# sony/aki

Hardware: AMD Instinct MI355X
Metric: image+text tokens/sec forward, AKI-4B, 336px img + 512 txt (higher is better)
Workload: dtype bf16

## Files before the change

### aki_amd/build.py

```python
from __future__ import annotations

import argparse
import concurrent.futures as cf
import os
import subprocess
import sys

PKG = os.path.dirname(os.path.abspath(__file__))
ROOT = os.path.dirname(PKG)
CSRC = os.path.join(PKG, "csrc")
LIBDIR = os.path.join(PKG, "lib")
LIB = os.path.join(LIBDIR, "libaki_mi355x.so")
LAB_LIB = os.path.join(LIBDIR, "libaki_mi355x_lab.so")
LAB_SOURCES = ["api.hip", "gemm_bf16.hip", "gemm_tn_bf16.hip", "mma_attn_bf16.hip", "mma_attn64_bf16.hip", "decode_chain.hip"]
LAB_ONLY_SOURCES = []
SOURCES = ["api.hip", "gemm_bf16.hip", "gemm_tn_bf16.hip", "mma_attn_bf16.hip", "mma_attn64_bf16.hip", "attn_nc_bf16.hip", "decode.hip", "decode_chain.hip", "train_kernels.hip", "attn_bwd_bf16.hip", "fp8_quant.hip", "simple_f32.hip", "aux_kernels.hip", "stack.hip"]
ARCH = "gfx950"
FILE_FLAGS = {"mma_attn64_bf16.hip": ["-fno-slp-vectorize"]}


def csrc_hash() -> str:
    import hashlib
    h = hashlib.sha256()
    files = sorted(os.path.join(CSRC, f) for f in os.listdir(CSRC) if f.endswith((".hip", ".h"))) + [os.path.join(ROOT, "include", "aki_mi355x.h")]
    for f in files:
        h.update(os.path.basename(f).encode())
        h.update(open(f, "rb").read())
    return h.hexdigest()[:16]


def _hipcc() -> str:
    for c in (os.environ.get("HIPCC"), "/opt/rocm/bin/hipcc", "hipcc"):
        if c and (os.path.isabs(c) and os.path.exists(c) or not os.path.isabs(c)):
            return c
    return "hipcc"


def _newer(target: str, deps) -> bool:
    if not os.path.exists(target):
        return False
    t = os.path.getmtime(target)
    return all(os.path.getmtime(d) <= t for d in deps)


def build(force: bool = False, save_temps: bool = False, verbose: bool = True, lab: bool = True) -> str:
    os.makedirs(LIBDIR, exist_ok=True)
    objdir = os.path.join(LIBDIR, "obj")
    os.makedirs(objdir, exist_ok=True)
    headers = [os.path.join(CSRC, "aki_device.h"), os.path.join(CSRC, "attn_mma_common.h"), os.path.join(ROOT, "include", "aki_mi355x.h")]
    srcs = [os.path.join(CSRC, s) for s in SOURCES]
    lab_only = [os.path.join(CSRC, s_) for s_ in LAB_ONLY_SOURCES]
    if not force and _newer(LIB, srcs + headers) and (not lab or _newer(LAB_LIB, srcs + lab_only + headers)):
        return LIB
    flags = [f"--offload-arch={ARCH}", "-O3", "-fPIC", "-std=c++17", "-I", os.path.join(ROOT, "include"), "-I", CSRC,
             "-Wno-unused-result", "-ffp-contract=off"]
    if save_temps:
        flags += ["-save-temps=obj", "-Rpass-analysis=kernel-resource-usage"]

    def cc(job):
        src, is_lab = job
        obj = os.path.join(objdir, os.path.basename(src).replace(".hip", ".lab.o" if is_lab else ".o"))
        if not force and _newer(obj, [src] + headers):
            return obj, ""
        extra = (["-DAKI_LAB_HOOKS"] if is_lab else []) + FILE_FLAGS.get(os.path.basename(src), [])
        r = subprocess.run([_hipcc()] + flags + extra + ["-c", src, "-o", obj], capture_output=True, text=True)
        if r.returncode != 0:
            raise RuntimeError(f"hipcc failed for {src}:\n{r.stdout}\n{r.stderr}")
        return obj, r.stderr

    jobs = [(s_, False) for s_ in srcs] + ([(os.path.join(CSRC, s_), True) for s_ in LAB_SOURCES + LAB_ONLY_SOURCES] if lab else [])
    with cf.ThreadPoolExecutor(max_workers=min(4, len(jobs))) as ex:
        results = list(ex.map(cc, jobs))
    objs = [o for o, _ in results[:len(srcs)]]
    lab_objs = [o for o, _ in results[len(srcs):]]
    if verbose:
        for _, log in results:
            if log.strip():
                sys.stderr.write(log)
    r = subprocess.run([_hipcc(), f"--offload-arch={ARCH}", "-shared", "-fPIC", "-o", LIB] + objs, capture_output=True, text=True)
    if r.returncode != 0:
        raise RuntimeError(f"link failed:\n{r.stdout}\n{r.stderr}")
    if lab:
        swapped = {os.path.basename(o).replace(".lab.o", ".o"): o for o in lab_objs}
        mix = [swapped.pop(os.path.basename(o), o) for o in objs] + list(swapped.values())
        r = subprocess.run([_hipcc(), f"--offload-arch={ARCH}", "-shared", "-fPIC", "-o", LAB_LIB] + mix, capture_output=True, text=True)
        if r.returncode != 0:
            raise RuntimeError(f"link (lab) failed:\n{r.stdout}\n{r.stderr}")
    return LIB


if __name__ == "__main__":
    ap = argparse.ArgumentParser()
    ap.add_argument("--force", action="store_true")
    ap.add_argument("--save-temps", action="store_true")
    ap.add_argument("--no-lab", action="store_true", help="skip libaki_mi355x_lab.so")
    a = ap.parse_args()
    print(build(force=a.force, save_temps=a.save_temps, lab=not a.no_lab))
```

### aki_amd/csrc/attn_mma_common.h

```cpp
#pragma once
#include <type_traits>

#include "aki_device.h"

namespace aki {

struct AttnParams {
  const bf16_t* q;
  const bf16_t* k;
  const bf16_t* v;
  bf16_t* o;
  float* lse;
  const aki_mma_rect* rects;
  const uint64_t* vbits;
  const int* seq_lens;
  int max_rects;
  int B, H, L;
  int nqt, nwords;
  int splits;
  int group_bh;
  int kvcap;
  float scale_log2;
  int dead_uniform;
};

constexpr int KROW = 192;
constexpr int VROW = 192;
constexpr int KTILE = 64 * KROW;
constexpr int VTILE = 64 * VROW;
constexpr int NSTAGE = 3;

constexpr int MAX_VB_WORDS = 256;

__device__ __forceinline__ float max3(float a, float b, float c) {
  float r;
  asm("v_max3_f32 %0, %1, %2, %3" : "=v"(r) : "v"(a), "v"(b), "v"(c));
  return r;
}

__device__ __forceinline__ float tile_max32(const f32x16& s0, const f32x16& s1) {
  float m, m1, m2, m3;
  asm("v_max3_f32 %0, %4, %5, %6\n\tv_max3_f32 %1, %7, %8, %9\n\tv_max3_f32 %2, %10, %11, %12\n\tv_max3_f32 %3, %13, %14, %15\n\t"
      "v_max3_f32 %0, %0, %16, %17\n\tv_max3_f32 %1, %1, %18, %19\n\tv_max3_f32 %2, %2, %20, %21\n\tv_max3_f32 %3, %3, %22, %23"
      : "=&v"(m), "=&v"(m1), "=&v"(m2), "=&v"(m3)
      : "v"(s0[0]), "v"(s0[1]), "v"(s1[0]), "v"(s0[4]), "v"(s0[5]), "v"(s1[4]), "v"(s0[8]), "v"(s0[9]), "v"(s1[8]), "v"(s0[12]), "v"(s0[13]), "v"(s1[12]),
        "v"(s1[1]), "v"(s0[2]), "v"(s1[5]), "v"(s0[6]), "v"(s1[9]), "v"(s0[10]), "v"(s1[13]), "v"(s0[14]));
  asm("v_max3_f32 %0, %0, %4, %5\n\tv_max3_f32 %1, %1, %6, %7\n\tv_max3_f32 %2, %2, %8, %9\n\tv_max3_f32 %3, %3, %10, %11\n\t"
      "v_max3_f32 %0, %0, %12, %13\n\tv_max3_f32 %2, %2, %14, %15\n\tv_max3_f32 %0, %0, %1, %2\n\tv_max_f32 %0, %0, %3"
      : "+v"(m), "+v"(m1), "+v"(m2), "+v"(m3)
      : "v"(s0[3]), "v"(s1[2]), "v"(s0[7]), "v"(s1[6]), "v"(s0[11]), "v"(s1[10]), "v"(s0[15]), "v"(s1[14]),
        "v"(s1[3]), "v"(s1[7]), "v"(s1[11]), "v"(s1[15]));
  return m;
}

__device__ __forceinline__ int count_le(int x) {
  const int n = 4 * (x >> 3) + min((x & 7) + 1, 4);
  return x < 0 ? 0 : min(n, 32);
}

__device__ __forceinline__ unsigned low_bits(int n) { return n >= 32 ? ~0u : ((1u << n) - 1u); }

template <int BIT>
__device__ __forceinline__ float mask_bias(int hid, int ninf) {
  float b;
  asm("v_bfe_i32 %0, %1, %2, 1\n\tv_and_b32 %0, %3, %0" : "=&v"(b) : "v"(hid), "n"(BIT), "s"(ninf));
  return b;
}

template <int BIT0, int BIT1>
__device__ __forceinline__ void mask_bias2(int hid, int ninf, float& b0, float& b1) {
  asm volatile("v_bfe_i32 %0, %2, %3, 1\n\tv_bfe_i32 %1, %2, %4, 1\n\tv_and_b32 %0, %5, %0\n\tv_and_b32 %1, %5, %1"
               : "=&v"(b0), "=&v"(b1) : "v"(hid), "n"(BIT0), "n"(BIT1), "s"(ninf));
}

template <int N, class F>
__device__ __forceinline__ void static_for(F&& f) {
  if constexpr (N > 0) {
    static_for<N - 1>(f);
    f(std::integral_constant<int, N - 1>{});
  }
}

template <int OFF>
__device__ __forceinline__ u32x2 ds_read_tr(unsigned lds_addr) {
  u32x2 r;
  asm volatile("ds_read_b64_tr_b16 %0, %1 offset:%2" : "=v"(r) : "v"(lds_addr), "n"(OFF));
  return r;
}

}
```

### aki_amd/csrc/mma_attn64_bf16.hip

```cpp
#include "attn_mma_common.h"

namespace aki {

constexpr int A64_O = 64;
constexpr int A64_Q = 160;
constexpr int A64_KA = 208;
constexpr int A64_KC = 232;
constexpr int A64_L = 56;

template <int R> __device__ __forceinline__ void acc_zero() { asm volatile("v_accvgpr_write_b32 a%c0, 0" ::"n"(R)); }
template <int R> __device__ __forceinline__ void acc_set(unsigned x) { asm volatile("v_accvgpr_write_b32 a%c1, %0" ::"v"(x), "n"(R)); }
template <int R> __device__ __forceinline__ float acc_get() {
  float x;
  asm volatile("v_accvgpr_read_b32 %0, a%c1" : "=v"(x) : "n"(R));
  return x;
}
template <int R> __device__ __forceinline__ void acc_scale4(float alpha) {
  float t0, t1, t2, t3;
  asm volatile(
      "v_accvgpr_read_b32 %0, a%c5\n\tv_accvgpr_read_b32 %1, a%c6\n\tv_accvgpr_read_b32 %2, a%c7\n\tv_accvgpr_read_b32 %3, a%c8\n\t"
      "v_mul_f32 %0, %0, %4\n\tv_mul_f32 %1, %1, %4\n\tv_mul_f32 %2, %2, %4\n\tv_mul_f32 %3, %3, %4\n\t"
      "v_accvgpr_write_b32 a%c5, %0\n\tv_accvgpr_write_b32 a%c6, %1\n\tv_accvgpr_write_b32 a%c7, %2\n\tv_accvgpr_write_b32 a%c8, %3"
      : "=&v"(t0), "=&v"(t1), "=&v"(t2), "=&v"(t3)
      : "v"(alpha), "n"(R), "n"(R + 1), "n"(R + 2), "n"(R + 3));
// ... 246 lines not shown
  const float m = tile_max32(s0, s1);
  const float mx = halves_max(m) * c + X.hide;
  const float m_new = fmaxf(X.m_ref, mx);
  const float alpha = __builtin_amdgcn_exp2f(X.m_ref - m_new);
  const bool started = __ballot(X.m_ref > -1e29f) != 0ull;
  X.m_ref = m_new;
  if (started) {
    {
      float lt;
      asm volatile("v_accvgpr_read_b32 %0, a%c2\n\ts_nop 0\n\tv_mul_f32 %0, %0, %1\n\ts_nop 0\n\tv_accvgpr_write_b32 a%c2, %0" : "=&v"(lt) : "v"(alpha), "n"(A64_L + 4 * ((OA - A64_O) / 48)));
    }
    static_for<12>([&](auto I) { acc_scale4<OA + 4 * decltype(I)::value>(alpha); });
  }
  const float nm = -m_new + X.hide;
#pragma unroll
  for (int r = 0; r < 16; r += 2) {
    const float a = __builtin_amdgcn_exp2f(__builtin_fmaf(s0[r], c, nm)), b = __builtin_amdgcn_exp2f(__builtin_fmaf(s0[r + 1], c, nm));
    const float d = __builtin_amdgcn_exp2f(__builtin_fmaf(s1[r], c, nm)), e = __builtin_amdgcn_exp2f(__builtin_fmaf(s1[r + 1], c, nm));
    const unsigned w0 = pack_bf16x2(a, b), w1 = pack_bf16x2(d, e);
    pin(w0, w1);
    pf[r >> 3][(r & 7) >> 1] = w0;
    pf[2 + (r >> 3)][(r & 7) >> 1] = w1;
  }
}
template <int THR, int ABL>
__global__ __launch_bounds__(256, 1) void mma_attn64_bf16_kernel(const AttnParams p) {
  constexpr int NT = 256;
  constexpr int OROW = 208;
  constexpr int LDS_RING = NSTAGE * KTILE + NSTAGE * VTILE, LDS_VB = MAX_VB_WORDS * 8, LDS_OUT = 8 * 32 * OROW;
  __shared__ __attribute__((aligned(16))) char smem[LDS_RING + LDS_VB + LDS_OUT + 16];
  char* const sK = smem;
  char* const sV = smem + NSTAGE * KTILE;
  const unsigned sVB_a = (unsigned)(unsigned long)((__attribute__((address_space(3))) char*)(smem + NSTAGE * KTILE + NSTAGE * VTILE));
  if constexpr (THR != 0) asm volatile("" ::: "a56", "a57", "a58", "a59", "a60", "a61", "a62", "a63");
  asm volatile("" ::: "a64", "a65", "a66", "a67", "a68", "a69", "a70", "a71", "a72", "a73", "a74", "a75", "a76", "a77", "a78", "a79", "a80", "a81", "a82", "a83", "a84", "a85", "a86", "a87", "a88", "a89", "a90", "a91", "a92", "a93", "a94", "a95", "a96", "a97", "a98", "a99", "a100", "a101", "a102", "a103", "a104", "a105", "a106", "a107", "a108", "a109", "a110", "a111", "a112", "a113", "a114", "a115", "a116", "a117", "a118", "a119", "a120", "a121", "a122", "a123", "a124", "a125", "a126", "a127", "a128", "a129", "a130", "a131", "a132", "a133", "a134", "a135", "a136", "a137", "a138", "a139", "a140", "a141", "a142", "a143", "a144", "a145", "a146", "a147", "a148", "a149", "a150", "a151", "a152", "a153", "a154", "a155", "a156", "a157", "a158", "a159", "a160", "a161", "a162", "a163", "a164", "a165", "a166", "a167", "a168", "a169", "a170", "a171", "a172", "a173", "a174", "a175", "a176", "a177", "a178", "a179", "a180", "a181", "a182", "a183", "a184", "a185", "a186", "a187", "a188", "a189", "a190", "a191", "a192", "a193", "a194", "a195", "a196", "a197", "a198", "a199", "a200", "a201", "a202", "a203", "a204", "a205", "a206", "a207", "a208", "a209", "a210", "a211", "a212", "a213", "a214", "a215", "a216", "a217", "a218", "a219", "a220", "a221", "a222", "a223", "a224", "a225", "a226", "a227", "a228", "a229", "a230", "a231", "a232", "a233", "a234", "a235", "a236", "a237", "a238", "a239", "a240", "a241", "a242", "a243", "a244", "a245", "a246", "a247", "a248", "a249", "a250", "a251", "a252", "a253", "a254", "a255");

  const int tid = threadIdx.x, lane = tid & 63;
  const int wave = __builtin_amdgcn_readfirstlane(tid >> 6);
  const int l31 = lane & 31, h = lane >> 5;
  const unsigned ones_w = (((lane & 7) == 0 && ((lane >> 4) & 1) == 0) || ((lane & 7) == 4 && ((lane >> 4) & 1) == 1)) ? 0x3f803f80u : 0u;
  const u32x4 sel = {ones_w, ones_w, ones_w, ones_w};
  const unsigned sFlag_a = (unsigned)(unsigned long)((__attribute__((address_space(3))) char*)(smem + LDS_RING + LDS_VB + LDS_OUT));
  if constexpr (THR != 0) {
    if (tid == 0) { *(unsigned*)(smem + LDS_RING + LDS_VB + LDS_OUT) = 0u; *(unsigned*)(smem + LDS_RING + LDS_VB + LDS_OUT + 4) = 0u; }
  }
  bool force_checked = false;
  int vpar = 0;

  const int grp = blockIdx.x / (p.group_bh * p.splits);
  const int bh0 = grp * p.group_bh;
  const int gbh = min(p.group_bh, p.B * p.H - bh0);
  const int within = blockIdx.x - bh0 * p.splits;
  const int sidx = within / gbh;
  const int bh = bh0 + within - sidx * gbh;
  const int b = bh / p.H, head = bh - b * p.H;
  const int L = p.L;
  const bf16_t* qb = p.q + ((size_t)bh * L) * 96;
  const char* kb = (const char*)(p.k + ((size_t)bh * p.kvcap) * 96);
  const char* vb_ = (const char*)(p.v + ((size_t)bh * p.kvcap) * 96);
  const int Lb = p.seq_lens ? min(p.seq_lens[b], L) : L;

  int d_ko[3];
#pragma unroll
  for (int i = 0; i < 3; ++i) {
    const int ch = i * NT + tid;
    const int kr = ch / 12, pos = ch - kr * 12;
    d_ko[i] = kr * 192 + (pos ^ ((kr >> 2) & 3)) * 16;
  }
  const int d_vo = tid * 16;
  const __amdgpu_buffer_rsrc_t rsrc_k = __builtin_amdgcn_make_buffer_rsrc((void*)kb, 0, L * 192, 0x00020000);
  const __amdgpu_buffer_rsrc_t rsrc_v = __builtin_amdgcn_make_buffer_rsrc((void*)vb_, 0, L * 192, 0x00020000);
  auto dma_k = [&](auto I, int t, int st) {
    constexpr int i = decltype(I)::value;
    if constexpr (ABL & 2) return;
    __builtin_amdgcn_raw_ptr_buffer_load_lds(rsrc_k, AKI_LDS_PTR(sK + st * KTILE + (i * NT + wave * 64) * 16), 16, d_ko[i], t * 12288, 0, 0);
  };
  auto dma_v = [&](auto I, int t, int st) {
    constexpr int i = decltype(I)::value;
    if constexpr (ABL & 2) return;
    __builtin_amdgcn_raw_ptr_buffer_load_lds(rsrc_v, AKI_LDS_PTR(sV + st * VTILE + (i * NT + wave * 64) * 16), 16, d_vo, t * 12288 + i * 4096, 0, 0);
  };

  int first_bad = 0x7fffffff;
  {
    unsigned long long bad = 0ull;
    int base = 0;
#pragma unroll
    for (int q4 = 3; q4 >= 0; --q4) {
      const int w = lane + 64 * q4;
      unsigned long long vbw = ~0ull;
      if (w < p.nwords) {
        if (p.vbits) vbw = p.vbits[(size_t)b * p.nwords + w];
        else vbw = (w * 64 + 64 <= L) ? ~0ull : ((1ull << (L - w * 64)) - 1ull);
        if (wave == 0) *(unsigned long long*)(smem + NSTAGE * KTILE + NSTAGE * VTILE + 8 * w) = vbw;
      }
      const unsigned long long m = __ballot(vbw != ~0ull);
      if (m != 0ull) { bad = m; base = 64 * q4; }
    }
    if (bad != 0ull) first_bad = base + __builtin_ctzll(bad);
    __syncthreads();
  }
  auto valid_word = [&](int w) -> unsigned long long {
    const unsigned addr = sVB_a + 8u * (unsigned)min(w, p.nwords - 1);
    u32x2 r;
    asm volatile("ds_read_b64 %0, %1\n\ts_waitcnt lgkmcnt(0)" : "=v"(r) : "v"(addr) : "memory");
    const unsigned lo = __builtin_amdgcn_readfirstlane(r[0]), hi = __builtin_amdgcn_readfirstlane(r[1]);
    return ((unsigned long long)hi << 32) | lo;
  };

  u32x4 rect_reg = {0u, 0u, 0u, 0u};
  if (lane < p.max_rects) rect_reg = *(const u32x4*)(p.rects + (size_t)b * p.max_rects + lane);
  const unsigned long long rv_ = __ballot(rect_reg[1] > rect_reg[0] && rect_reg[3] > rect_reg[2]);
  const int nrect = rv_ == 0ull ? 0 : 64 - (int)__builtin_clzll(rv_);
  auto rect_at = [&](int i) -> aki_mma_rect {
    aki_mma_rect o;
    o.row_lo = (int)__builtin_amdgcn_readlane(rect_reg[0], i); o.row_hi = (int)__builtin_amdgcn_readlane(rect_reg[1], i);
    o.col_lo = (int)__builtin_amdgcn_readlane(rect_reg[2], i); o.col_hi = (int)__builtin_amdgcn_readlane(rect_reg[3], i);
    return o;
  };
  auto block_extent = [&](int r0) -> int {
    if (r0 >= L) return -1;
    int ext = min(r0 + 32, L);
    for (int i = 0; i < nrect; ++i) {
      const aki_mma_rect r = rect_at(i);
      if (r.row_hi > r.row_lo && r.col_hi > r.col_lo && r.row_lo < r0 + 32 && r.row_hi > r0) ext = max(ext, min(r.col_hi, L));
    }
    if (p.dead_uniform && min(r0 + 32, L) > Lb) ext = L;
    return ext;
  };
  const int nblk = (L + 31) >> 5;
  const bool sched = nblk <= 128;
  int er0 = 0xff, er1 = 0xff;
  if (sched) {
    const int ext0 = block_extent(32 * lane);
    const int ext1 = block_extent(32 * (lane + 64));
    const int key0 = ext0 < 0 ? -1 : ext0 * 256 + lane;
    const int key1 = ext1 < 0 ? -1 : ext1 * 256 + lane + 64;
    int r0 = 0, r1 = 0;
    for (int i = 0; i < 64; ++i) {
      const int k0 = __builtin_amdgcn_readlane(key0, i), k1 = __builtin_amdgcn_readlane(key1, i);
      r0 += (k0 > key0 ? 1 : 0) + (k1 > key0 ? 1 : 0);
      r1 += (k0 > key1 ? 1 : 0) + (k1 > key1 ? 1 : 0);
    }
    er0 = ext0 >= 0 ? (ext0 << 8) | r0 : 0xff;
    er1 = ext1 >= 0 ? (ext1 << 8) | r1 : 0xff;
  }
  auto ranked_block = [&](int R, int& wq0, int& ext) {
    wq0 = L; ext = 0;
    const unsigned long long m0 = __ballot((er0 & 0xff) == R);
    const unsigned long long m1 = __ballot((er1 & 0xff) == R);
    if (m0 != 0ull) {
      const int l = __builtin_ctzll(m0);
      wq0 = 32 * l; ext = __builtin_amdgcn_readlane(er0, l) >> 8;
    } else if (m1 != 0ull) {
      const int l = __builtin_ctzll(m1);
      wq0 = 32 * (l + 64); ext = __builtin_amdgcn_readlane(er1, l) >> 8;
    }
  };

  const int kswz = (l31 >> 2) & 3;
  const int k_even = l31 * KROW + ((h ^ kswz) << 4);
  const int k_odd = l31 * KROW + (((2 + h) ^ kswz) << 4);
  const int voff = (4 * h + ((lane & 15) >> 2)) * VROW + (16 * ((lane >> 4) & 1) + 4 * (lane & 3)) * 2;
  const unsigned sK_a = (unsigned)(unsigned long)((__attribute__((address_space(3))) char*)sK);
  const unsigned sV_a = (unsigned)(unsigned long)((__attribute__((address_space(3))) char*)sV);
  const float c = p.scale_log2;
  const float rc = 1.0f / c;

  unsigned long long st_pro = 0, st_loop = 0, st_epi = 0, st_tiles = 0, st_t = 0, st_rt0 = 0, st_redo = 0, st_wait = 0, st_dma = 0;
  unsigned long long st_h[4] = {0, 0, 0, 0}, st_n = 0, st_slow = 0, st_nslow = 0, st_full = 0;
  if constexpr (ABL & 512) { st_rt0 = __builtin_amdgcn_s_memrealtime(); }

  struct { int wq0A, wq0B, jendA, jendB, jend; } nx = {0, 0, 0, 0, 0};
  auto rank_of = [&](int kk) -> int { return kk * p.splits + ((kk & 1) ? p.splits - 1 - sidx : sidx); };
  auto prefetch_rank = [&](int g) {
    int wq0A = L, wq0B = L, extA = 0, extB = 0, hi_col = 0;
    if (sched) {
#pragma unroll
      for (int w = 0; w < 4; ++w) {
        int wa, ea, wb, eb;
// ... 303 lines not shown
    if constexpr (ABL & 512) tw0 = __builtin_amdgcn_s_memtime();
    if constexpr (ABL & 1024) tit0 = __builtin_amdgcn_s_memtime();
    if constexpr (!(ABL & 2)) asm volatile("s_waitcnt vmcnt(6)" ::: "memory");
    if constexpr (ABL & 512) { const unsigned long long t_ = __builtin_amdgcn_s_memtime(); st_dma += t_ - tw0; tw0 = t_; }
    if constexpr (!(ABL & 8)) __builtin_amdgcn_s_barrier();
    if constexpr (ABL & 512) st_wait += __builtin_amdgcn_s_memtime() - tw0;
    A64_PIN();
    const int tk = j + 3, tv = j + 2;
    auto dma_e = [&](auto I) { if constexpr (THR == 0 && decltype(I)::value < 3) dma_k(I, tk, st0); };
    auto dma_o = [&](auto I) {
      constexpr int i = decltype(I)::value;
      if constexpr (THR == 0) { if constexpr (i < 3) dma_v(I, tv, st2); }
      else if constexpr (i < 3) dma_k(I, tk, st0);
      else if constexpr (i < 6) dma_v(std::integral_constant<int, i - 3>{}, tv, st2);
    };
    const unsigned va = sV_a + st0 * VTILE + voff;
    const unsigned ke = sK_a + st1 * KTILE + k_even, ko = sK_a + st1 * KTILE + k_odd;
    unsigned long long th_ = 0;
    if constexpr ((ABL & 1024) && ft) th_ = __builtin_amdgcn_s_memtime();
    constexpr bool gap_bias = THR != 0 && (mode == 0 || mode == 4 || mode == 7);
    using GB = std::integral_constant<bool, gap_bias>;
    int hidY = 0;
    float hideY = 0.f;
    if constexpr (gap_bias) bias_hid(B, j, hidY, hideY);
    half1(BL{}, T_{}, BB{}, GB{}, sB0, sB1, hidY, sA0, sA1, pA, A, tA, uA, pB, va, dma_e);
    if constexpr ((ABL & 1024) && ft) { const unsigned long long t_ = __builtin_amdgcn_s_memtime(); st_h[0] += t_ - th_; th_ = t_; }
    if constexpr (gap_bias) { B.hide = hideY; asm volatile("s_nop 1" : "+v"(sB0), "+v"(sB1)); }
    else if constexpr (mode == 1) fast_hide(B, j); else if constexpr (mode != 2) tile_bias(B, j, sB0, sB1);
    A64_PIN();
    half2(BL{}, T_{}, BB{}, FT{}, sB0, sB1, sA0, sA1, pA, A, tA, uA, ke, ko);
    if constexpr ((ABL & 1024) && ft) { const unsigned long long t_ = __builtin_amdgcn_s_memtime(); st_h[1] += t_ - th_; }
    wait_v_frags();
    asm volatile("s_nop 1" : "+v"(pA[0]), "+v"(pA[1]), "+v"(pA[2]), "+v"(pA[3]));
    A64_PIN();
    if constexpr ((ABL & 1024) && ft) th_ = __builtin_amdgcn_s_memtime();
    if constexpr (gap_bias) bias_hid(A, j + 1, hidY, hideY);
    half1(BL{}, F_{}, BA{}, GB{}, sA0, sA1, hidY, sB0, sB1, pB, B, tB, uB, pA, va, dma_o);
    if constexpr ((ABL & 1024) && ft) { const unsigned long long t_ = __builtin_amdgcn_s_memtime(); st_h[2] += t_ - th_; th_ = t_; }
    if constexpr (!(ABL & 4)) asm volatile("s_waitcnt lgkmcnt(0)" ::: "memory");
    A64_PIN();
    if constexpr (gap_bias) { A.hide = hideY; asm volatile("s_nop 1" : "+v"(sA0), "+v"(sA1)); }
    else if constexpr (mode == 1) fast_hide(A, j + 1); else if constexpr (mode != 2) tile_bias(A, j + 1, sA0, sA1);
    A64_PIN();
    half2(BL{}, F_{}, BA{}, FT{}, sA0, sA1, sB0, sB1, pB, B, tB, uB, ke, ko);
    if constexpr ((ABL & 1024) && ft) { const unsigned long long t_ = __builtin_amdgcn_s_memtime(); st_h[3] += t_ - th_; st_n += 1; }
    asm volatile("s_nop 1" : "+v"(pB[0]), "+v"(pB[1]), "+v"(pB[2]), "+v"(pB[3]));
    A64_PIN();
    const int t_ = st0; st0 = st1; st1 = st2; st2 = t_;
    if constexpr ((ABL & 1024) && !ft) { st_slow += __builtin_amdgcn_s_memtime() - tit0; st_nslow += 1; }
    if constexpr ((ABL & 1024) && ft) st_full += __builtin_amdgcn_s_memtime() - tit0;
  };
  auto both_fast = [&](int j) -> bool {
    const int t = j & 63;
    return t != 63 && ((B.fast >> t) & (A.fast >> (t + 1)) & 1ull) != 0ull;
  };
  bool settled = (THR == 0 || (ABL & 1)) && !(ABL & 64);
  int j = 0;
  while (j < jend_w) {
    const int t = j & 63;
    int nrun = 0;
    if constexpr (THR != 0) {
      if (settled) {
        const unsigned long long mR = (B.fast & (A.fast >> 1)) >> t;
        nrun = min(min(mR == ~0ull ? 64 : (int)__builtin_ctzll(~mR), 63 - t), jend_w - j);
        if (nrun > 0) {
          nrun = min(nrun, min(const_len(B, j), const_len(A, j + 1)));
          const float hA1 = hide_val(A, j + 1);
          if (__ballot(hA1 != A.hide) != 0ull) nrun = 0;
          if (nrun > 0) B.hide = hide_val(B, j);
        }
      }
    }
    if (__builtin_expect(nrun > 0, 1)) {
      if (nrun & 1) { iter(M2{}, j); ++j; --nrun; }
      while (nrun > 0) { iter(M2{}, j); iter(M2{}, j + 1); j += 2; nrun -= 2; }
    } else if (THR == 0 && both_fast(j)) {
      do { iter(M1{}, j); ++j; } while (j < jend_w && both_fast(j));
    } else if (THR == 0 || settled) {
      iter(M0{}, j); ++j;
    } else {
      if constexpr (THR != 0) { if (j == 0 && !force_checked && !(ABL & 64)) iter(M7{}, j); else iter(M4{}, j); }
      ++j;
      if constexpr (THR != 0) {
        if (!settled && !force_checked && !(ABL & 64))
          settled = __ballot((A.m_ref < -1e29f && (A.row_alive || A.row_uniform)) || (B.m_ref < -1e29f && (B.row_alive || B.row_uniform))) == 0ull;
      }
    }
    if ((j & 63) == 0) { block_masks(A, j); block_masks(B, j); }
  }
  for (; j < jend; ++j) {
    if constexpr (!(ABL & 2)) asm volatile("s_waitcnt vmcnt(6)" ::: "memory");
    if constexpr (!(ABL & 8)) __builtin_amdgcn_s_barrier();
    const int tk = j + 3, tv = j + 2;
    static_for<3>([&](auto I) { dma_k(I, tk, st0); });
    static_for<3>([&](auto I) { dma_v(I, tv, st2); });
    const int t_ = st0; st0 = st1; st1 = st2; st2 = t_;
  }
  if (jend_w > 0) {
    static_for<12>([&](auto I) {
      constexpr int i = decltype(I)::value, ks4 = i / 3, dt = i % 3;
      const u32x4 vv = {vlo[ks4][dt][0], vlo[ks4][dt][1], vhi[ks4][dt][0], vhi[ks4][dt][1]};
      mfma_pv<A64_O + 48 + 16 * dt>(vv, pB[ks4]);
      if constexpr (THR != 0 && dt == 2) mfma_ones<A64_L + 4>(sel, pB[ks4]);
    });
  }
  asm volatile("s_waitcnt vmcnt(0)" ::: "memory");
  bool walk_again = false;
  if constexpr (THR != 0) {
    asm volatile("s_nop 15" ::: "memory");
    const float lA = acc_get<A64_L>(), lB = acc_get<A64_L + 4>();
    const bool bad = !force_checked && __ballot(!(lA < 0x1p64f) || !(lB < 0x1p64f)) != 0ull;
    const unsigned fa_ = sFlag_a + 4u * (unsigned)vpar, one = 1u, zero = 0u;
    if (bad) asm volatile("ds_write_b32 %0, %1" ::"v"(fa_), "v"(one) : "memory");
    asm volatile("s_waitcnt lgkmcnt(0)" ::: "memory");
    __builtin_amdgcn_s_barrier();
    unsigned fl;
    asm volatile("ds_read_b32 %0, %1\n\ts_waitcnt lgkmcnt(0)" : "=v"(fl) : "v"(fa_) : "memory");
    walk_again = __builtin_amdgcn_readfirstlane(fl) != 0u;
    const unsigned fo_ = sFlag_a + 4u * (unsigned)(vpar ^ 1);
    if (wave == 0) asm volatile("ds_write_b32 %0, %1" ::"v"(fo_), "v"(zero) : "memory");
    vpar ^= 1;
  } else {
    __builtin_amdgcn_s_barrier();
  }
  if (walk_again) {
    force_checked = true;
    prefetch_rank(g);
    --kk;
    continue;
  }
  force_checked = false;
  if (rank_of(kk + 1) < p.nqt) prefetch_rank(rank_of(kk + 1));
  if constexpr (ABL & 512) { const unsigned long long t_ = __builtin_amdgcn_s_memtime(); st_loop += t_ - st_t; st_t = t_; st_redo += A.l_dbg + B.l_dbg; }
  asm volatile("s_nop 15\n\ts_nop 15" ::: "memory");
  A64_PIN();

  int lane_o = lane;
  asm volatile("" : "+v"(lane_o));
  const int l31_o = lane_o & 31, h_o = lane_o >> 5;
  const unsigned sO_a = (unsigned)(unsigned long)((__attribute__((address_space(3))) char*)(smem + LDS_RING + LDS_VB));
  auto store_block = [&](auto XB, A64Blk& X) {
    constexpr int xb = decltype(XB)::value;
    float l_tot;
    if constexpr (THR != 0) l_tot = acc_get<A64_L + 4 * xb>();
    else l_tot = halves_sum(X.l);
    const bool dead = !(l_tot > 0.f);
    const unsigned sO = sO_a + (unsigned)((wave * 2 + xb) * (32 * OROW));
    const float inv = dead ? 0.f : 1.0f / l_tot;
    static_for<12>([&](auto I) {
      constexpr int i = decltype(I)::value, dt = i / 4, q4 = i % 4;
      float v[4];
      v[0] = acc_get<A64_O + 48 * xb + 16 * dt + 4 * q4 + 0>() * inv;
      v[1] = acc_get<A64_O + 48 * xb + 16 * dt + 4 * q4 + 1>() * inv;
      v[2] = acc_get<A64_O + 48 * xb + 16 * dt + 4 * q4 + 2>() * inv;
      v[3] = acc_get<A64_O + 48 * xb + 16 * dt + 4 * q4 + 3>() * inv;
      if (dead && p.dead_uniform && X.row < L) {
        float a0 = 0.f, a1 = 0.f, a2 = 0.f, a3 = 0.f;
        const char* vp = vb_ + (dt * 32 + q4 * 8 + 4 * h_o) * 2;
        for (int t2 = 0; t2 < L; ++t2) {
          const u32x2 w2 = *(const u32x2*)(vp + (size_t)t2 * 192);
          a0 += bf16_lo(w2[0]); a1 += bf16_hi(w2[0]); a2 += bf16_lo(w2[1]); a3 += bf16_hi(w2[1]);
        }
        const float il = 1.0f / (float)L;
        v[0] = a0 * il; v[1] = a1 * il; v[2] = a2 * il; v[3] = a3 * il;
      }
      const u32x2 pk = {pack_bf16x2(v[0], v[1]), pack_bf16x2(v[2], v[3])};
      const unsigned wa = sO + (unsigned)(l31_o * OROW + (dt * 32 + q4 * 8 + 4 * h_o) * 2);
      asm volatile("ds_write_b64 %0, %1" ::"v"(wa), "v"(pk) : "memory");
    });
    asm volatile("s_waitcnt lgkmcnt(0)" ::: "memory");
    bf16_t* const obase = p.o + ((size_t)b * L * p.H + head) * 96;
#pragma unroll
    for (int it = 0; it < 6; ++it) {
      const int ch = it * 64 + lane_o;
      const int r = ch / 12, cc = ch - r * 12;
      u32x4 w4;
      const unsigned ra_ = sO + (unsigned)(r * OROW + cc * 16);
      asm volatile("ds_read_b128 %0, %1\n\ts_waitcnt lgkmcnt(0)" : "=&v"(w4) : "v"(ra_) : "memory");
      if (X.wq0 + r < L) *(u32x4*)((char*)(obase + (size_t)(X.wq0 + r) * p.H * 96) + cc * 16) = w4;
    }
    if (!(ABL & 512) && p.lse && h_o == 0 && X.row < L) p.lse[(size_t)bh * L + X.row] = dead ? -INFINITY : (X.m_ref + __builtin_amdgcn_logf(l_tot)) * 0.69314718055994530942f;
  };
  store_block(BA{}, A);
  store_block(BB{}, B);
  if constexpr (ABL & 512) { const unsigned long long t_ = __builtin_amdgcn_s_memtime(); st_epi += t_ - st_t; }
  }
  if constexpr (ABL & 512) {
    if (p.lse && tid == 0) {
      float* d = p.lse + 8 * blockIdx.x;
      d[0] = (float)st_pro; d[1] = (float)st_loop; d[2] = (float)st_epi; d[3] = (float)st_tiles;
      d[4] = (float)(__builtin_amdgcn_s_memrealtime() - st_rt0);
      d[5] = (float)st_redo;
      d[6] = (float)st_dma;
      d[7] = (float)st_wait;
      if constexpr (ABL & 1024) { d[0] = (float)st_h[0]; d[1] = (float)st_h[1]; d[2] = (float)st_h[2]; d[5] = (float)st_h[3]; d[3] = (float)st_n; d[6] = (float)st_slow; d[7] = (float)st_nslow; d[4] = (float)st_full; }
    }
  }
#undef A64_PIN
}

#ifdef AKI_LAB_HOOKS
extern int g_attn_variant;
#endif

int attn_core64_bf16_launch(AttnParams p, int cus, hipStream_t stream, int exact_max) {
  const int nbh = p.B * p.H;
  p.nqt = (p.L + 255) / 256;
  int splits = (cus + nbh - 1) / nbh;
  p.splits = splits < 1 ? 1 : (splits > p.nqt ? p.nqt : splits);
  int grp = ((cus + p.splits - 1) / p.splits + 7) & ~7;
  p.group_bh = grp > nbh ? nbh : grp;
#ifdef AKI_LAB_HOOKS
#define A64_ABL_CASE(m) if (g_attn_variant == 100 + (m)) { hipLaunchKernelGGL((mma_attn64_bf16_kernel<8, (m)>), dim3(nbh * p.splits), dim3(256), 0, stream, p); return AKI_OK; }
  A64_ABL_CASE(64) A64_ABL_CASE(512) A64_ABL_CASE(513) A64_ABL_CASE(514) A64_ABL_CASE(515) A64_ABL_CASE(520) A64_ABL_CASE(521) A64_ABL_CASE(523) A64_ABL_CASE(1536) A64_ABL_CASE(1537)
#undef A64_ABL_CASE
#endif
  if (exact_max) hipLaunchKernelGGL((mma_attn64_bf16_kernel<0, 0>), dim3(nbh * p.splits), dim3(256), 0, stream, p);
  else hipLaunchKernelGGL((mma_attn64_bf16_kernel<8, 0>), dim3(nbh * p.splits), dim3(256), 0, stream, p);
  return AKI_OK;
}

}
```

### aki_amd/csrc/mma_attn_bf16.hip

```cpp
#include "attn_mma_common.h"

#ifndef AKI_ATTN_L2_ROWS
#define AKI_ATTN_L2_ROWS 256
#endif
#ifndef AKI_ATTN_SCHED_MAX
#define AKI_ATTN_SCHED_MAX 64
#endif

namespace aki {

template <int NW, int MODE>
__global__ __launch_bounds__(NW * 64, 2) void mma_attn_bf16_kernel(const AttnParams p) {
  constexpr bool SWP = MODE == 1 || MODE == 2;
  static_assert(MODE != 2 || NW == 8, "the ping-pong loop is written for two groups of four waves");
  constexpr int BQ = NW * 32;
  constexpr int NT = NW * 64;
  constexpr int NCH = (64 * 12 + NT - 1) / NT;
  __shared__ __attribute__((aligned(16))) char smem[NSTAGE * KTILE + NSTAGE * VTILE + MAX_VB_WORDS * 8 + (MODE == 4 ? 64 : 0)];
  char* const sK = smem;
  char* const sV = smem + NSTAGE * KTILE;
  unsigned long long* const sVB = (unsigned long long*)(smem + NSTAGE * KTILE + NSTAGE * VTILE);
  unsigned* const sCnt = (unsigned*)(smem + NSTAGE * KTILE + NSTAGE * VTILE + MAX_VB_WORDS * 8);

  const int tid = threadIdx.x, lane = tid & 63;
// ... 449 lines not shown
      u32x2 vlo[4][3], vhi[4][3];
      {
        const unsigned vaddr = (unsigned)(unsigned long)((__attribute__((address_space(3))) char*)sV) + stage * VTILE + voff;
        static_for<4>([&](auto ks4) {
          static_for<3>([&](auto dt) {
            constexpr int off = ks4 * 16 * VROW + dt * 64;
            vlo[ks4][dt] = ds_read_tr<off>(vaddr);
            vhi[ks4][dt] = ds_read_tr<off + 8 * VROW>(vaddr);
          });
        });
      }
      __builtin_amdgcn_sched_barrier(0);
      mfma_results_settle(s0, s1);
      float mx = tile_max32(s0, s1);
      mx = halves_max(mx) * p.scale_log2;
      const float m_new = fmaxf(m_run, mx);
      const bool moved = m_new != m_run;
      const float alpha = __builtin_amdgcn_exp2f(m_run - m_new);
      m_run = m_new;
      float ps = 0.f;
#pragma unroll
      for (int r = 0; r < 16; ++r) {
        s0[r] = __builtin_amdgcn_exp2f(__builtin_fmaf(s0[r], p.scale_log2, -m_new));
        s1[r] = __builtin_amdgcn_exp2f(__builtin_fmaf(s1[r], p.scale_log2, -m_new));
        ps += s0[r] + s1[r];
      }
      l_part = l_part * alpha + ps;
      if (__any(moved)) {
#pragma unroll
        for (int dt = 0; dt < 3; ++dt)
#pragma unroll
          for (int r = 0; r < 16; ++r) o[dt][r] *= alpha;
      }

      asm volatile("s_waitcnt lgkmcnt(0)"
                   : "+v"(vlo[0][0]), "+v"(vhi[0][0]), "+v"(vlo[0][1]), "+v"(vhi[0][1]), "+v"(vlo[0][2]), "+v"(vhi[0][2]),
                     "+v"(vlo[1][0]), "+v"(vhi[1][0]), "+v"(vlo[1][1]), "+v"(vhi[1][1]), "+v"(vlo[1][2]), "+v"(vhi[1][2]),
                     "+v"(vlo[2][0]), "+v"(vhi[2][0]), "+v"(vlo[2][1]), "+v"(vhi[2][1]), "+v"(vlo[2][2]), "+v"(vhi[2][2]),
                     "+v"(vlo[3][0]), "+v"(vhi[3][0]), "+v"(vlo[3][1]), "+v"(vhi[3][1]), "+v"(vlo[3][2]), "+v"(vhi[3][2]));
      __builtin_amdgcn_sched_barrier(0);
      if constexpr (MODE == 4) {
        if (lane == 0) __hip_atomic_fetch_add(sCnt + NSTAGE + stage, 1u, __ATOMIC_RELAXED, __HIP_MEMORY_SCOPE_WORKGROUP);
      }
#pragma unroll
      for (int ks4 = 0; ks4 < 4; ++ks4) {
        bf16x8 pf;
#pragma unroll
        for (int e = 0; e < 8; ++e) pf[e] = (__bf16)((ks4 < 2) ? s0[8 * (ks4 & 1) + e] : s1[8 * (ks4 & 1) + e]);
#pragma unroll
        for (int dt = 0; dt < 3; ++dt) {
          const u32x4 vv = {vlo[ks4][dt][0], vlo[ks4][dt][1], vhi[ks4][dt][0], vhi[ks4][dt][1]};
          o[dt] = __builtin_amdgcn_mfma_f32_32x32x16_bf16(__builtin_bit_cast(bf16x8, vv), pf, o[dt], 0, 0, 0);
        }
      }
    } else {
      if constexpr (MODE == 4) {
        if (lane == 0) __hip_atomic_fetch_add(sCnt + NSTAGE + stage, 1u, __ATOMIC_RELAXED, __HIP_MEMORY_SCOPE_WORKGROUP);
      }
      if (DMA_LATE && j + 2 < jend) {
        if constexpr (MODE == 4) {
          if (j >= 1) {
            const unsigned wantf = (unsigned)NW * (unsigned)((j - 1) / NSTAGE + 1);
            while (__hip_atomic_load(sCnt + NSTAGE + dma_stage, __ATOMIC_RELAXED, __HIP_MEMORY_SCOPE_WORKGROUP) < wantf) { }
          }
        }
        issue_tile(j + 2, dma_stage);
      }
    }
    vb_next = valid_word(j + 1);
    if (++stage == NSTAGE) stage = 0;
  }

  }
  const float l_tot = halves_sum(l_part);
  const bool dead = !(l_tot > 0.f);
  __syncthreads();
  if constexpr (MODE == 4) {
    if (tid < 2 * NSTAGE) sCnt[tid] = 0u;
  }
  constexpr int OROW = 208;
  char* const sO = sK + wave * (32 * OROW);
  {
    const float inv = dead ? 0.f : 1.0f / l_tot;
#pragma unroll
    for (int dt = 0; dt < 3; ++dt)
#pragma unroll
      for (int q4 = 0; q4 < 4; ++q4) {
        float v[4];
#pragma unroll
        for (int e = 0; e < 4; ++e) v[e] = o[dt][4 * q4 + e] * inv;
        if (dead && p.dead_uniform && row < L) {
          float a0 = 0.f, a1 = 0.f, a2 = 0.f, a3 = 0.f;
          const char* vp = vb_ + (dt * 32 + q4 * 8 + 4 * h) * 2;
          for (int t2 = 0; t2 < L; ++t2) {
            const u32x2 w2 = *(const u32x2*)(vp + (size_t)t2 * 192);
            a0 += bf16_lo(w2[0]); a1 += bf16_hi(w2[0]); a2 += bf16_lo(w2[1]); a3 += bf16_hi(w2[1]);
          }
          const float il = 1.0f / (float)L;
          v[0] = a0 * il; v[1] = a1 * il; v[2] = a2 * il; v[3] = a3 * il;
        }
        const u32x2 pk = {pack_bf16x2(v[0], v[1]), pack_bf16x2(v[2], v[3])};
        *(u32x2*)(sO + l31 * OROW + (dt * 32 + q4 * 8 + 4 * h) * 2) = pk;
      }
  }
  bf16_t* const obase = p.o + ((size_t)b * L * p.H + head) * 96;
#pragma unroll
  for (int it = 0; it < 6; ++it) {
    const int ch = it * 64 + lane_o;
    const int r = ch / 12, c = ch - r * 12;
    const u32x4 w4 = *(const u32x4*)(sO + r * OROW + c * 16);
    if (wq0 + r < L) *(u32x4*)((char*)(obase + (size_t)(wq0 + r) * p.H * 96) + c * 16) = w4;
  }
  if (p.lse && h == 0 && row < L) p.lse[(size_t)bh * L + row] = dead ? -INFINITY : (m_run + __builtin_amdgcn_logf(l_tot)) * 0.69314718055994530942f;
  __syncthreads();
  }
}

int attn_core64_bf16_launch(AttnParams p, int cus, hipStream_t stream, int exact_max);
#ifndef AKI_ATTN64_MIN_L
#define AKI_ATTN64_MIN_L 1792
#endif

#ifdef AKI_LAB_HOOKS
int g_attn_variant = 0;
#endif

int attn_core_bf16(const aki_mma_attn_core_args* a, void* ws, size_t ws_bytes, hipStream_t stream) {
  if (a->Dh != 96) return AKI_ERR_UNSUPPORTED;
  if (a->max_rects < 0 || a->max_rects > AKI_MAX_RECTS) return AKI_ERR_INVALID_ARG;
  if ((a->L + 63) / 64 > MAX_VB_WORDS) return AKI_ERR_UNSUPPORTED;
  AKI_CHECK_ALIGN16(a->q); AKI_CHECK_ALIGN16(a->k); AKI_CHECK_ALIGN16(a->v); AKI_CHECK_ALIGN16(a->o);
  (void)ws; (void)ws_bytes;
  constexpr int NW = 4;
  AttnParams p = {};
  p.q = (const bf16_t*)a->q; p.k = (const bf16_t*)a->k; p.v = (const bf16_t*)a->v; p.o = (bf16_t*)a->o; p.lse = a->lse;
  p.rects = a->rects; p.vbits = a->col_valid_bits; p.seq_lens = a->seq_lens;
  p.max_rects = a->rects ? a->max_rects : 0;
  p.B = a->B; p.H = a->H; p.L = a->L;
  p.nqt = (a->L + NW * 32 - 1) / (NW * 32);
  p.nwords = (a->L + 63) / 64;
  {
    static int cus = 0;
    if (cus == 0) {
      int dev = 0, n = 0;
      if (hipGetDevice(&dev) != hipSuccess || hipDeviceGetAttribute(&n, hipDeviceAttributeMultiprocessorCount, dev) != hipSuccess || n <= 0) n = 256;
      cus = n;
    }
    const int nbh = a->B * a->H;
    int splits = (2 * cus + nbh - 1) / nbh;
#ifdef AKI_ATTN_SPLITS
    splits = AKI_ATTN_SPLITS;
#endif
#ifdef AKI_LAB_HOOKS
    if (g_attn_variant == 6) splits = 1;
    if (g_attn_variant == 7) splits = 3;
#endif
    const int s_l2 = a->L / AKI_ATTN_L2_ROWS;
    if (splits < s_l2) splits = s_l2;
    p.splits = splits < 1 ? 1 : (splits > p.nqt ? p.nqt : splits);
    int grp = ((2 * cus + p.splits - 1) / p.splits + 7) & ~7;
    p.group_bh = grp > nbh ? nbh : grp;
  }
  p.kvcap = a->kv_capacity > 0 ? a->kv_capacity : a->L;
  if (p.kvcap < a->L) return AKI_ERR_INVALID_ARG;
  p.scale_log2 = a->scale * 1.44269504088896340736f;
  p.dead_uniform = a->dead_rows == AKI_DEAD_ROWS_UNIFORM;
  AKI_CLEAR_ERR();
  {
    bool long_core = a->L >= AKI_ATTN64_MIN_L;
    int exact_max = 0;
#ifdef AKI_LAB_HOOKS
    if (g_attn_variant >= 1 && g_attn_variant <= 8) long_core = false;
    if (g_attn_variant == 9 || g_attn_variant == 10 || g_attn_variant > 100) { long_core = true; exact_max = g_attn_variant == 10; }
#endif
    if (long_core) {
      static int cus64 = 0;
      if (cus64 == 0) {
        int dev = 0, n = 0;
        if (hipGetDevice(&dev) != hipSuccess || hipDeviceGetAttribute(&n, hipDeviceAttributeMultiprocessorCount, dev) != hipSuccess || n <= 0) n = 256;
        cus64 = n;
      }
      const int rc = attn_core64_bf16_launch(p, cus64, stream, exact_max);
// ... 35 lines not shown
```

Baseline: 132,900.

## Cooperatively compute V-mean for dead rows and settle early on fully masked prefixes

Dead rows under dead_uniform used to compute the mean of V with each lane serially looping over all L keys for every one of its 12 output chunks. That loop is replaced by a wave-cooperative V-mean: 48 lanes each stride over a quarter of the keys in 16-byte chunks, reduce with shuffles, and every lane then picks its values by shuffle. The 64-wide kernel also finds the first valid key column from the valid bitmask and lets rows that can see nothing before it stop blocking the early 'settled' check. The build script adds an assembly audit step for the attn64 kernel, which uses -save-temps on every compile of that file.

Result: no change. 132,800, median of 6 (-0.1%).

```diff
diff --git a/aki_amd/build.py b/aki_amd/build.py
--- a/aki_amd/build.py
+++ b/aki_amd/build.py
@@ -17,6 +17,25 @@
 SOURCES = ["api.hip", "gemm_bf16.hip", "gemm_tn_bf16.hip", "mma_attn_bf16.hip", "mma_attn64_bf16.hip", "attn_nc_bf16.hip", "decode.hip", "decode_chain.hip", "train_kernels.hip", "attn_bwd_bf16.hip", "fp8_quant.hip", "simple_f32.hip", "aux_kernels.hip", "stack.hip"]
 ARCH = "gfx950"
 FILE_FLAGS = {"mma_attn64_bf16.hip": ["-fno-slp-vectorize"]}
+AUDITED = {"mma_attn64_bf16.hip": (None, ("ILi0ELi0E", "ILi8ELi0E", "ILi8ELi64E"))}
+
+
+def _audit(src: str, asm_dir: str, is_lab: bool) -> None:
+    import contextlib
+    import importlib.util
+    import io
+    spec = importlib.util.spec_from_file_location("attn64_audit", os.path.join(ROOT, "tools", "attn64_audit.py"))
+    mod = importlib.util.module_from_spec(spec)
+    spec.loader.exec_module(mod)
+    s_files = [f for f in os.listdir(asm_dir) if f.endswith("gfx950.s")]
+    if len(s_files) != 1:
+        raise RuntimeError(f"no device assembly of {src} in {asm_dir} to audit")
+    log = io.StringIO()
+    with contextlib.redirect_stdout(log):
+        bad = mod.audit_s(os.path.join(asm_dir, s_files[0]), AUDITED[os.path.basename(src)][1 if is_lab else 0])
+    if bad:
+        raise RuntimeError(f"{os.path.basename(src)}{' (lab)' if is_lab else ''}: the accumulator-register / scratch / hazard audit "
+                           f"failed - the asm statements' register map is no longer safe with this compiler:\n{log.getvalue()}")
 
 
 def csrc_hash() -> str:
@@ -63,9 +82,25 @@
         if not force and _newer(obj, [src] + headers):
             return obj, ""
         extra = (["-DAKI_LAB_HOOKS"] if is_lab else []) + FILE_FLAGS.get(os.path.basename(src), [])
-        r = subprocess.run([_hipcc()] + flags + extra + ["-c", src, "-o", obj], capture_output=True, text=True)
+        audited = os.path.basename(src) in AUDITED
+        asm_dir = os.path.join(objdir, os.path.basename(src).replace(".hip", ".lab.asm" if is_lab else ".asm"))
+        fl = flags
+        if audited:
+            os.makedirs(asm_dir, exist_ok=True)
+            for f in os.listdir(asm_dir):
+                os.remove(os.path.join(asm_dir, f))
+            fl = [f for f in flags if not f.startswith("-save-temps")] + ["-save-temps"]
+        if os.path.exists(obj):
+            os.remove(obj)
+        r = subprocess.run([_hipcc()] + fl + extra + ["-c", src, "-o", obj], capture_output=True, text=True, cwd=asm_dir if audited else None)
         if r.returncode != 0:
             raise RuntimeError(f"hipcc failed for {src}:\n{r.stdout}\n{r.stderr}")
+        if audited:
+            try:
+                _audit(src, asm_dir, is_lab)
+            except Exception:
+                os.remove(obj)
+                raise
         return obj, r.stderr
 
     jobs = [(s_, False) for s_ in srcs] + ([(os.path.join(CSRC, s_), True) for s_ in LAB_SOURCES + LAB_ONLY_SOURCES] if lab else [])
diff --git a/aki_amd/csrc/attn_mma_common.h b/aki_amd/csrc/attn_mma_common.h
--- a/aki_amd/csrc/attn_mma_common.h
+++ b/aki_amd/csrc/attn_mma_common.h
@@ -88,4 +88,32 @@
   return r;
 }
 
+__device__ __forceinline__ void v_mean_chunks(const char* vb, int L, int lane, float (&m)[8]) {
+  const int c = lane % 12, r = lane / 12;
+#pragma unroll
+  for (int e = 0; e < 8; ++e) m[e] = 0.f;
+  if (r < 4) {
+#pragma unroll 8
+    for (int t = r; t < L; t += 4) {
+      const u32x4 w = *(const u32x4*)(vb + (size_t)t * 192 + c * 16);
+      m[0] += bf16_lo(w[0]); m[1] += bf16_hi(w[0]); m[2] += bf16_lo(w[1]); m[3] += bf16_hi(w[1]);
+      m[4] += bf16_lo(w[2]); m[5] += bf16_hi(w[2]); m[6] += bf16_lo(w[3]); m[7] += bf16_hi(w[3]);
+    }
+  }
+  const float il = 1.0f / (float)L;
+#pragma unroll
+  for (int e = 0; e < 8; ++e) {
+    m[e] += __shfl_down(m[e], 24);
+    m[e] += __shfl_down(m[e], 12);
+    m[e] *= il;
+  }
 }
+__device__ __forceinline__ void v_mean_pick(const float (&m)[8], int cc, int h, float (&v)[4]) {
+#pragma unroll
+  for (int e = 0; e < 4; ++e) {
+    const float lo = __shfl(m[e], cc), hi = __shfl(m[4 + e], cc);
+    v[e] = h ? hi : lo;
+  }
+}
+
+}
diff --git a/aki_amd/csrc/mma_attn64_bf16.hip b/aki_amd/csrc/mma_attn64_bf16.hip
--- a/aki_amd/csrc/mma_attn64_bf16.hip
+++ b/aki_amd/csrc/mma_attn64_bf16.hip
@@ -352,6 +352,7 @@
   };
 
   int first_bad = 0x7fffffff;
+  int first_valid = L;
   {
     unsigned long long bad = 0ull;
     int base = 0;
@@ -366,6 +367,12 @@
       }
       const unsigned long long m = __ballot(vbw != ~0ull);
       if (m != 0ull) { bad = m; base = 64 * q4; }
+      const unsigned long long mv = __ballot(w < p.nwords && vbw != 0ull);
+      if (mv != 0ull) {
+        const int lv = __builtin_ctzll(mv);
+        const unsigned lo = __builtin_amdgcn_readlane((unsigned)vbw, lv), hi = __builtin_amdgcn_readlane((unsigned)(vbw >> 32), lv);
+        first_valid = 64 * (lv + 64 * q4) + __builtin_ctzll(((unsigned long long)hi << 32) | lo);
+      }
     }
     if (bad != 0ull) first_bad = base + __builtin_ctzll(bad);
     __syncthreads();
@@ -835,8 +842,11 @@
       if constexpr (THR != 0) { if (j == 0 && !force_checked && !(ABL & 64)) iter(M7{}, j); else iter(M4{}, j); }
       ++j;
       if constexpr (THR != 0) {
-        if (!settled && !force_checked && !(ABL & 64))
-          settled = __ballot((A.m_ref < -1e29f && (A.row_alive || A.row_uniform)) || (B.m_ref < -1e29f && (B.row_alive || B.row_uniform))) == 0ull;
+        auto waits = [&](const A64Blk& X) {
+          const bool sees_nothing = X.row < first_valid && X.rc1 <= first_valid;
+          return X.m_ref < -1e29f && ((X.row_alive && !sees_nothing) || X.row_uniform);
+        };
+        if (!settled && !force_checked && !(ABL & 64)) settled = __ballot(waits(A) || waits(B)) == 0ull;
       }
     }
     if ((j & 63) == 0) { block_masks(A, j); block_masks(B, j); }
@@ -900,6 +910,10 @@
     const bool dead = !(l_tot > 0.f);
     const unsigned sO = sO_a + (unsigned)((wave * 2 + xb) * (32 * OROW));
     const float inv = dead ? 0.f : 1.0f / l_tot;
+    const bool mean_row = dead && p.dead_uniform && X.row < L;
+    const bool any_mean = __ballot(mean_row) != 0ull;
+    float vm[8] = {};
+    if (any_mean) v_mean_chunks(vb_, L, lane_o, vm);
     static_for<12>([&](auto I) {
       constexpr int i = decltype(I)::value, dt = i / 4, q4 = i % 4;
       float v[4];
@@ -907,15 +921,10 @@
       v[1] = acc_get<A64_O + 48 * xb + 16 * dt + 4 * q4 + 1>() * inv;
       v[2] = acc_get<A64_O + 48 * xb + 16 * dt + 4 * q4 + 2>() * inv;
       v[3] = acc_get<A64_O + 48 * xb + 16 * dt + 4 * q4 + 3>() * inv;
-      if (dead && p.dead_uniform && X.row < L) {
-        float a0 = 0.f, a1 = 0.f, a2 = 0.f, a3 = 0.f;
-        const char* vp = vb_ + (dt * 32 + q4 * 8 + 4 * h_o) * 2;
-        for (int t2 = 0; t2 < L; ++t2) {
-          const u32x2 w2 = *(const u32x2*)(vp + (size_t)t2 * 192);
-          a0 += bf16_lo(w2[0]); a1 += bf16_hi(w2[0]); a2 += bf16_lo(w2[1]); a3 += bf16_hi(w2[1]);
-        }
-        const float il = 1.0f / (float)L;
-        v[0] = a0 * il; v[1] = a1 * il; v[2] = a2 * il; v[3] = a3 * il;
+      if (any_mean) {
+        float u[4];
+        v_mean_pick(vm, 4 * dt + q4, h_o, u);
+        if (mean_row) { v[0] = u[0]; v[1] = u[1]; v[2] = u[2]; v[3] = u[3]; }
       }
       const u32x2 pk = {pack_bf16x2(v[0], v[1]), pack_bf16x2(v[2], v[3])};
       const unsigned wa = sO + (unsigned)(l31_o * OROW + (dt * 32 + q4 * 8 + 4 * h_o) * 2);
diff --git a/aki_amd/csrc/mma_attn_bf16.hip b/aki_amd/csrc/mma_attn_bf16.hip
--- a/aki_amd/csrc/mma_attn_bf16.hip
+++ b/aki_amd/csrc/mma_attn_bf16.hip
@@ -555,6 +555,10 @@
   char* const sO = sK + wave * (32 * OROW);
   {
     const float inv = dead ? 0.f : 1.0f / l_tot;
+    const bool mean_row = dead && p.dead_uniform && row < L;
+    const bool any_mean = __ballot(mean_row) != 0ull;
+    float vm[8] = {};
+    if (any_mean) v_mean_chunks(vb_, L, lane, vm);
 #pragma unroll
     for (int dt = 0; dt < 3; ++dt)
 #pragma unroll
@@ -562,15 +566,10 @@
         float v[4];
 #pragma unroll
         for (int e = 0; e < 4; ++e) v[e] = o[dt][4 * q4 + e] * inv;
-        if (dead && p.dead_uniform && row < L) {
-          float a0 = 0.f, a1 = 0.f, a2 = 0.f, a3 = 0.f;
-          const char* vp = vb_ + (dt * 32 + q4 * 8 + 4 * h) * 2;
-          for (int t2 = 0; t2 < L; ++t2) {
-            const u32x2 w2 = *(const u32x2*)(vp + (size_t)t2 * 192);
-            a0 += bf16_lo(w2[0]); a1 += bf16_hi(w2[0]); a2 += bf16_lo(w2[1]); a3 += bf16_hi(w2[1]);
-          }
-          const float il = 1.0f / (float)L;
-          v[0] = a0 * il; v[1] = a1 * il; v[2] = a2 * il; v[3] = a3 * il;
+        if (any_mean) {
+          float u[4];
+          v_mean_pick(vm, 4 * dt + q4, h, u);
+          if (mean_row) { v[0] = u[0]; v[1] = u[1]; v[2] = u[2]; v[3] = u[3]; }
         }
         const u32x2 pk = {pack_bf16x2(v[0], v[1]), pack_bf16x2(v[2], v[3])};
         *(u32x2*)(sO + l31 * OROW + (dt * 32 + q4 * 8 + 4 * h) * 2) = pk;
```
